# Hfx-J/SGTD

Hardware: AMD Instinct MI355X
Metric: query frames/sec vs map size (descriptor build + candidate selection) (higher is better)
Workload: dtype f64

## Files before the change

### sgtd_amd/csrc/select_kernels.hip.h

```cpp
#pragma once
#include "probe_kernels.hip.h"

#define SGTD_VT_THREADS 1024
#define SGTD_VT_BINS 4096
__host__ __device__ __forceinline__ size_t votes_topk_lds_bytes(u32 frame_span) {
  return (((size_t)frame_span + 3) & ~(size_t)3) * 4 + SGTD_VT_BINS * 4 + SGTD_TOPK_POOL * 8;
}

__global__ __launch_bounds__(SGTD_VT_THREADS) void votes_topk_kernel(QueryView Q, ProbeBuffers B, u32 frame_span, u32 frame_lo,
                                                                      int blocks_per_query, int cand_num, u32 *q_M,
                                                                      unsigned long long *q_P, int *n_cand, int *cand_frame,
                                                                      int *cand_votes, long long *pair_off, u32 *q_pairs) {
  constexpr int NW = SGTD_VT_THREADS / SGTD_WAVE;
  extern __shared__ u32 s_dyn[];
  u32 *s_hist = s_dyn;
  u32 *s_vb = s_dyn + ((frame_span + 3u) & ~3u);
  u64 *s_pool = reinterpret_cast<u64 *>(s_vb + SGTD_VT_BINS);
  __shared__ u32 s_pre[NW][32];
  __shared__ u32 s_ptr[NW][32];
  __shared__ u32 s_cnt[NW][32];
  __shared__ u32 s_M, s_thr, s_n_ge, s_npool;
  __shared__ unsigned long long s_P;
  __shared__ u64 s_red[NW];
  __shared__ int s_picked;
// ... 14 lines not shown
    }
    if (lane == 0) {
      atomicAdd(&s_M, total);
      atomicAdd(&s_P, (unsigned long long)visits);
    }
  }
  __syncthreads();
  u32 *votes = B.votes + (size_t)q * frame_span;
  for (u32 f = tid; f < frame_span; f += SGTD_VT_THREADS) {
    const u32 v = s_hist[f];
    votes[f] = v;
    if (v >= 5) atomicAdd(&s_vb[min(v, (u32)SGTD_VT_BINS - 1u)], 1u);
  }
  if (tid == 0) {
    atomicAdd(&q_M[q], s_M);
    atomicAdd(&q_P[q], s_P);
  }
  __syncthreads();
  if (tid < SGTD_WAVE) {
    constexpr int PER = SGTD_VT_BINS / SGTD_WAVE;
    u32 mine = 0;
    for (int b = 0; b < PER; b++) mine += s_vb[lane * PER + b];
    u32 suffix = mine;
#pragma unroll
    for (int d = 1; d < SGTD_WAVE; d <<= 1) {
      const u32 o = __shfl_down(suffix, d);
      if (lane + d < SGTD_WAVE) suffix += o;
    }
    const u64 okmask = __ballot(suffix >= (u32)cand_num);
    const u32 n_ge = __shfl(suffix, 0);
    if (okmask) {
      const int L = 63 - __builtin_clzll(okmask);
      if (lane == L) {
        u32 acc = suffix - mine;
        int b = L * PER + PER - 1;
        for (; b >= L * PER; b--) { acc += s_vb[b]; if (acc >= (u32)cand_num) break; }
        s_thr = (u32)max(b, 5); s_n_ge = acc;
      }
    } else if (lane == 0) { s_thr = 5; s_n_ge = n_ge; }
  }
  __syncthreads();
  const u32 thr = s_thr;
  int *cf = cand_frame + (size_t)q * cand_num, *cv = cand_votes + (size_t)q * cand_num;
  long long *po = pair_off + (size_t)q * (cand_num + 1);
  if (s_n_ge <= (u32)SGTD_TOPK_POOL) {
    for (u32 f = tid; f < frame_span; f += SGTD_VT_THREADS) {
      const u32 v = s_hist[f];
      if (v >= thr) s_pool[atomicAdd(&s_npool, 1u)] = ((u64)v << 32) | (u64)(0xFFFFFFFFu - f);
    }
    __syncthreads();
    if (tid < SGTD_WAVE) {
      constexpr int PER = SGTD_TOPK_POOL / SGTD_WAVE;
      const u32 np = s_npool;
      u64 a[PER];
#pragma unroll
      for (int k = 0; k < PER; k++) a[k] = ((u32)(k * SGTD_WAVE + lane) < np) ? s_pool[k * SGTD_WAVE + lane] : 0ull;
      int picked = 0;
      u32 acc = 0;
      for (int round = 0; round < cand_num; round++) {
        u64 best = 0;
#pragma unroll
        for (int k = 0; k < PER; k++) best = a[k] > best ? a[k] : best;
#pragma unroll
        for (int dlt = SGTD_WAVE / 2; dlt > 0; dlt >>= 1) {
          const u64 o = __shfl_xor(best, dlt);
          best = o > best ? o : best;
        }
        if ((u32)(best >> 32) < 5u) break;
#pragma unroll
        for (int k = 0; k < PER; k++) a[k] = (a[k] == best) ? 0ull : a[k];
        if (lane == 0) {
          const u32 f = 0xFFFFFFFFu - (u32)(best & 0xFFFFFFFFu);
          cf[picked] = (int)(f + frame_lo);
          cv[picked] = (int)(u32)(best >> 32);
          po[picked] = (long long)acc;
        }
        acc += (u32)(best >> 32);
        picked++;
      }
      if (lane == 0) {
        n_cand[q] = picked;
        q_pairs[q] = acc;
        for (int k = picked; k < cand_num; k++) { cf[k] = -1; cv[k] = 0; }
        for (int k = picked; k <= cand_num; k++) po[k] = (long long)acc;
      }
    }
    return;
  }
  u32 acc = 0;
  for (int round = 0; round < cand_num; round++) {
    u64 best = 0;
    for (u32 f = tid; f < frame_span; f += SGTD_VT_THREADS) {
      const u64 key = ((u64)s_hist[f] << 32) | (u64)(0xFFFFFFFFu - f);
      best = key > best ? key : best;
    }
#pragma unroll
    for (int dlt = SGTD_WAVE / 2; dlt > 0; dlt >>= 1) {
      const u64 o = __shfl_xor(best, dlt);
      best = o > best ? o : best;
    }
    if (lane == 0) s_red[wid] = best;
    __syncthreads();
    if (tid == 0) {
      u64 b = s_red[0];
      for (int w = 1; w < NW; w++) b = s_red[w] > b ? s_red[w] : b;
      const u32 v = (u32)(b >> 32);
      if (v >= 5) {
        const u32 f = 0xFFFFFFFFu - (u32)(b & 0xFFFFFFFFu);
        s_hist[f] = 0;
        cf[s_picked] = (int)(f + frame_lo);
        cv[s_picked] = (int)v;
        po[s_picked] = (long long)acc;
        acc += v;
        s_picked++;
      } else {
        s_picked |= 0x40000000;
      }
    }
    __syncthreads();
    if (s_picked & 0x40000000) break;
  }
  if (tid == 0) {
    const int picked = s_picked & 0x3FFFFFFF;
    n_cand[q] = picked;
    q_pairs[q] = acc;
    for (int k = picked; k < cand_num; k++) { cf[k] = -1; cv[k] = 0; }
    for (int k = picked; k <= cand_num; k++) po[k] = (long long)acc;
  }
}

__global__ __launch_bounds__(256) void cand_prefix_kernel(const int *n_cand, const int *cand_votes, int cand_num, int n_queries,
                                                          long long *pair_off, u32 *q_pairs) {
  const int q = blockIdx.x * blockDim.x + threadIdx.x;
  if (q >= n_queries) return;
  const int nc = n_cand[q];
  u32 acc = 0;
  for (int k = 0; k <= cand_num; k++) {
    pair_off[(size_t)q * (cand_num + 1) + k] = (long long)acc;
    if (k < nc) acc += (u32)cand_votes[(size_t)q * cand_num + k];
  }
  q_pairs[q] = acc;
}

#ifndef SGTD_PQ_THREADS
#define SGTD_PQ_THREADS 512
#endif
#define SGTD_PQ_WAVES (SGTD_PQ_THREADS / SGTD_WAVE)
#ifndef SGTD_PQ_WORDS
#define SGTD_PQ_WORDS 4
#endif
#ifndef SGTD_PQ_OCC
#define SGTD_PQ_OCC 4
#endif
#define SGTD_PQ_TILE_QUADS (SGTD_PQ_WAVES * SGTD_PQ_WORDS * SGTD_WAVE)
#define SGTD_PQ_WAVE_RECS (SGTD_PQ_WORDS * SGTD_WAVE * 4)
#define SGTD_PQ_TILE_RECS (SGTD_PQ_WAVES * SGTD_PQ_WAVE_RECS)
#define SGTD_PQ_DESCS SGTD_PQ_THREADS
#define SGTD_PQ_RANK_BITS (SGTD_PQ_DESCS <= 512 ? 17 : 16)
static_assert(SGTD_PQ_DESCS <= 1024 && SGTD_MAX_CAND <= 64, "an image word holds 6 slot bits and 26 - RANK_BITS descriptor bits");
static_assert(SGTD_PQ_WAVE_RECS * 4 >= 4 * 64 * 8 && (SGTD_PQ_WAVES & (SGTD_PQ_WAVES - 1)) == 0 && SGTD_PQ_WAVES >= 2,
              "a wave's region of the image holds the ranking masks of four dense words; image positions rotate over a power of two of regions");

struct __attribute__((aligned(16))) PqList { u32 pre, first, n, desc; };

template <bool SLOT_TABLE>
__global__ __launch_bounds__(SGTD_PQ_THREADS) __attribute__((amdgpu_waves_per_eu(SGTD_PQ_OCC, SGTD_PQ_OCC))) void pairs_query_kernel(QueryView Q, ProbeBuffers B, const int *n_cand,
                                                                       const int *cand_frame, int cand_num,
                                                                       const long long *pair_off, const u32 *q_pair_base,
                                                                       u64 *pairs, IdMap map, u32 frame_span, u32 frame_lo,
                                                                       const u64 *keep) {
  constexpr int NW = SGTD_PQ_WAVES, QW = SGTD_PQ_WORDS;
  extern __shared__ __attribute__((aligned(16))) u32 s_img[];
  unsigned char *s_slot8 = reinterpret_cast<unsigned char *>(s_img + SGTD_PQ_TILE_RECS);
  __shared__ PqList s_ne[SGTD_PQ_DESCS];
  __shared__ u32 s_start[SGTD_PQ_DESCS + SGTD_WAVE + 8];
  __shared__ u32 s_cnt[NW][64];
  __shared__ u32 s_scan[NW + 1];
  __shared__ u64 s_cand[SGTD_CAND_HASH];
  if (B.overflow()[0] || B.overflow()[1]) return;
  const int tid = threadIdx.x, lane = lane_id(), wid = tid >> 6;
  const int q = blockIdx.x;
  const u32 cnt = Q.count[q];
  const int nc = n_cand[q];
  if (nc == 0 || cnt == 0) return;
  const u64 kept = keep ? keep[q] : ~0ull;
  if (kept == 0) return;
  if (SLOT_TABLE) {
    for (u32 f = tid; f < (((frame_span + 15u) & ~15u) + 16u) / 4u; f += SGTD_PQ_THREADS) reinterpret_cast<u32 *>(s_slot8)[f] = 0xFFFFFFFFu;
    __syncthreads();
    if (tid < nc && ((kept >> tid) & 1ull)) s_slot8[(u32)cand_frame[(size_t)q * cand_num + tid] - frame_lo] = (unsigned char)tid;
  } else {
    s_cand[tid & (SGTD_CAND_HASH - 1)] = SGTD_CAND_EMPTY;
    __syncthreads();
    if (tid < nc && ((kept >> tid) & 1ull)) {
      const u32 f = (u32)cand_frame[(size_t)q * cand_num + tid];
      u32 h = (f * 0x9E3779B1u) >> 24;
      while (atomicCAS(&s_cand[h], SGTD_CAND_EMPTY, ((u64)f << 8) | (u64)tid) != SGTD_CAND_EMPTY) h = (h + 1) & (SGTD_CAND_HASH - 1);
    }
  }
  u32 out_next = 0, first_of_slot = 0;
  if (lane < nc) {
    out_next = q_pair_base[q] + (u32)pair_off[(size_t)q * (cand_num + 1) + lane];
    first_of_slot = map.frame_first[(u32)cand_frame[(size_t)q * cand_num + lane] - map.frame_lo];
  }
  const u32 id_bits = B.id_bits, rank_mask = (1u << id_bits) - 1u;
  const u64 lane_bit = 1ull << lane;
  u32 *my_img = s_img + wid * SGTD_PQ_WAVE_RECS;
  for (u32 sb0 = 0; sb0 < cnt; sb0 += SGTD_PQ_DESCS) {
    __syncthreads();
    u32 n = 0, p = 0;
    if (sb0 + tid < cnt) {
      const uint2 lp = B.list[(long long)q * Q.stride + sb0 + tid];
      p = lp.x; n = lp.y;
    }
    u32 RQ, K;
    const u32 pre = block_excl_scan((n + 3u) >> 2, s_scan, RQ);
    const u32 kx = block_excl_scan(n ? 1u : 0u, s_scan, K);
    if (n) { s_ne[kx] = PqList{pre, p, n, (u32)tid}; s_start[kx] = pre; }
    if ((u32)tid >= K) s_start[tid] = 0xFFFFFFFFu;
    if (tid < SGTD_WAVE + 8) s_start[SGTD_PQ_DESCS + tid] = 0xFFFFFFFFu;
    static_assert(SGTD_PQ_THREADS >= SGTD_WAVE + 8, "the end markers behind the list starts are written by the first 72 threads");
    __syncthreads();
    if (RQ == 0) continue;
    const u32 n_tiles = (RQ + SGTD_PQ_TILE_QUADS - 1) / SGTD_PQ_TILE_QUADS;
    uint4 nrec[QW];
    u32 nk[QW], ndd[QW];
    auto fetch = [&](u32 t) {
      const u32 r0 = t * SGTD_PQ_TILE_QUADS + (u32)wid * (QW * SGTD_WAVE);
      u32 below = 0;
#pragma unroll
      for (int i = 0; i < SGTD_PQ_DESCS / SGTD_WAVE; i++) below += s_start[i * SGTD_WAVE + lane] <= r0 ? 1u : 0u;
      const u32 k0 = wave_sum(below) - 1u;
      const u32 st = s_start[k0 + 1u + (u32)lane];
      u32 kl[QW];
      u32 c_prev = 0;
      bool slow = false;
#pragma unroll
      for (int u = 0; u < QW; u++) {
        const u32 w_lo = r0 + (u32)u * SGTD_WAVE;
        const u32 c = (u32)__builtin_popcountll(__builtin_amdgcn_ballot_w64(st <= w_lo + SGTD_WAVE));
        u64 marks = 0;
        for (u32 i = c_prev; i < c; i++) marks |= 1ull << ((u32)__builtin_amdgcn_readlane((int)st, (int)i) - 1u - w_lo);
        kl[u] = k0 + c_prev + __builtin_amdgcn_mbcnt_hi((u32)(marks >> 32), __builtin_amdgcn_mbcnt_lo((u32)marks, 0u));
        c_prev = c;
        slow = slow || c >= (u32)SGTD_WAVE;
      }
      if (slow) {
#pragma unroll
        for (int u = 0; u < QW; u++) {
          const u32 r = r0 + (u32)u * SGTD_WAVE + (u32)lane;
          u32 lo = 0, hi = K;
          while (hi - lo > 1u) {
            const u32 mid = (lo + hi) >> 1;
            if (s_start[mid] <= r) lo = mid; else hi = mid;
          }
          kl[u] = lo;
        }
      }
#pragma unroll
      for (int u = 0; u < QW; u++) {
        const u32 r = r0 + (u32)u * SGTD_WAVE + (u32)lane;
        const PqList L = s_ne[min(kl[u], K - 1u)];
        const bool ok = r < RQ;
        const u32 quad = r - L.pre;
        nk[u] = ok ? min(4u, L.n - (quad << 2)) : 0u;
        ndd[u] = L.desc << SGTD_PQ_RANK_BITS;
        nrec[u] = *reinterpret_cast<const uint4 *>(B.rec_at(ok ? L.first + quad : 0u));
      }
    };
    fetch(0);
    for (u32 t = 0; t < n_tiles; t++) {
      uint4 rc[QW];
      u32 kk[QW], dd[QW];
#pragma unroll
      for (int u = 0; u < QW; u++) { rc[u] = nrec[u]; kk[u] = nk[u]; dd[u] = ndd[u]; }
      if (t + 1 < n_tiles) fetch(t + 1);
#if defined(SGTD_EXP_PQ) && SGTD_EXP_PQ == 2
      {
        u32 x = 0;
        for (int u = 0; u < QW; u++) x ^= rc[u].x ^ rc[u].y ^ rc[u].z ^ rc[u].w ^ kk[u] ^ dd[u];
        if (x == 0x12345678u) pairs[0] = x;
        continue;
      }
#endif
      u32 nd = 0;
      static_assert(QW % 2 == 0, "the candidates of two quad-words are counted by one wave scan (16-bit halves)");
#pragma unroll
      for (int u0 = 0; u0 < QW; u0 += 2) {
        u32 sl[2][4], mine[2] = {0, 0};
#pragma unroll
        for (int h = 0; h < 2; h++) {
          const int u = u0 + h;
          const u32 w4[4] = {rc[u].x, rc[u].y, rc[u].z, rc[u].w};
#pragma unroll
          for (int i = 0; i < 4; i++) {
            const u32 lf = w4[i] >> id_bits;
            if (SLOT_TABLE) {
              sl[h][i] = (u32)s_slot8[min(lf, frame_span)];
              sl[h][i] = (u32)i < kk[u] ? sl[h][i] : 0xFFu;
            } else {
              sl[h][i] = 0xFFu;
              if ((u32)i < kk[u] && lf < frame_span) sl[h][i] = cand_slot(s_cand, lf + frame_lo);
            }
            mine[h] += sl[h][i] != 0xFFu ? 1u : 0u;
          }
        }
        const u32 both = mine[0] | (mine[1] << 16);
        const u32 inc = wave_incl_scan(both);
        const u32 tot2 = (u32)__builtin_amdgcn_readlane((int)inc, SGTD_WAVE - 1);
        u32 at[2] = {nd + ((inc - both) & 0xFFFFu), nd + (tot2 & 0xFFFFu) + ((inc - both) >> 16)};
#pragma unroll
        for (int h = 0; h < 2; h++) {
          const int u = u0 + h;
          const u32 w4[4] = {rc[u].x, rc[u].y, rc[u].z, rc[u].w};
#pragma unroll
          for (int i = 0; i < 4; i++)
            if (sl[h][i] != 0xFFu) my_img[at[h]++] = (sl[h][i] << 26) | dd[u] | (w4[i] & rank_mask);
        }
        nd += (tot2 & 0xFFFFu) + (tot2 >> 16);
      }
#if defined(SGTD_EXP_PQ) && SGTD_EXP_PQ == 3
      if (nd == 0xFFFFFFFFu) pairs[0] = 0;
      continue;
#endif
      __builtin_amdgcn_wave_barrier();
      constexpr int MAXD = SGTD_PQ_WAVE_RECS / SGTD_WAVE, GRP = 4;
      u32 dw[MAXD], rk[MAXD];
      const u32 ndw = (nd + SGTD_WAVE - 1) / SGTD_WAVE;
#pragma unroll
      for (int g0 = 0; g0 < MAXD; g0 += GRP) {
#pragma unroll
        for (int w = g0; w < g0 + GRP; w++) { dw[w] = 0xFFFFFFFFu; rk[w] = 0; }
        if ((u32)g0 < ndw) {
#pragma unroll
          for (int w = g0; w < g0 + GRP; w++) {
            const u32 v = my_img[w * SGTD_WAVE + lane];
            dw[w] = (u32)(w * SGTD_WAVE + lane) < nd ? v : 0xFFFFFFFFu;
          }
        }
      }
      u32 run_s = 0;
      u64 *m = reinterpret_cast<u64 *>(my_img);
#pragma unroll
      for (int g0 = 0; g0 < MAXD; g0 += GRP) {
        if ((u32)g0 < ndw) {
          __builtin_amdgcn_wave_barrier();
#pragma unroll
          for (int w = 0; w < GRP; w++) m[w * SGTD_WAVE + lane] = 0;
          __builtin_amdgcn_wave_barrier();
#pragma unroll
          for (int w = 0; w < GRP; w++)
            if (dw[g0 + w] != 0xFFFFFFFFu) atomicOr(&m[w * SGTD_WAVE + (dw[g0 + w] >> 26)], lane_bit);
          __builtin_amdgcn_wave_barrier();
#pragma unroll
          for (int w = 0; w < GRP; w++) {
            const u64 own = m[w * SGTD_WAVE + lane];
            const u32 s = (dw[g0 + w] >> 26) & 63u;
            const u64 gm = m[w * SGTD_WAVE + s];
            const u32 before = (u32)__builtin_amdgcn_ds_bpermute((int)(s << 2), (int)run_s);
            rk[g0 + w] = before + __builtin_amdgcn_mbcnt_hi((u32)(gm >> 32), __builtin_amdgcn_mbcnt_lo((u32)gm, 0u));
            run_s += (u32)__builtin_popcountll(own);
          }
        }
      }
      s_cnt[wid][lane] = run_s;
      __syncthreads();
#if defined(SGTD_EXP_PQ) && SGTD_EXP_PQ == 4
      if (rk[0] == 0xFFFFFFF1u) pairs[0] = 0;
      continue;
#endif
      u32 tot = 0, mine_before = 0;
#pragma unroll
      for (int w = 0; w < NW; w++) {
        const u32 c = s_cnt[w][lane];
        mine_before += w < wid ? c : 0u;
        tot += c;
      }
      const u32 slot_inc = wave_incl_scan(tot);
      const u32 slot_off = slot_inc - tot;
      const u32 n_img = (u32)__builtin_amdgcn_readlane((int)slot_inc, SGTD_WAVE - 1);
      const u32 my_base = slot_off + mine_before;
#pragma unroll
      for (int g0 = 0; g0 < MAXD; g0 += GRP) {
        if ((u32)g0 < ndw) {
#pragma unroll
          for (int w = g0; w < g0 + GRP; w++) {
            const u32 pos = (u32)__builtin_amdgcn_ds_bpermute((int)((dw[w] >> 26) << 2), (int)my_base) + rk[w];
            if (dw[w] != 0xFFFFFFFFu)
              s_img[((pos >> 6) & (NW - 1)) * SGTD_PQ_WAVE_RECS + (((pos >> 6) / NW) << 6) + (pos & 63u)] = dw[w];
          }
        }
      }
      __syncthreads();
#if defined(SGTD_EXP_PQ) && SGTD_EXP_PQ == 5
      out_next += tot;
      continue;
#endif
      for (u32 c = (u32)wid; c * SGTD_WAVE < n_img; c += NW) {
        const u32 e = c * SGTD_WAVE + lane;
        const bool ok = e < n_img;
        const u32 wv = my_img[((c / NW) << 6) + lane];
        const u32 s4 = ok ? (wv >> 26) << 2 : 0u;
        const u32 o = (u32)__builtin_amdgcn_ds_bpermute((int)s4, (int)(out_next - slot_off));
        u32 g = (u32)__builtin_amdgcn_ds_bpermute((int)s4, (int)first_of_slot) + (wv & ((1u << SGTD_PQ_RANK_BITS) - 1u));
        if (ok) {
          if (map.by_frame) g = map.by_frame[g];
#if defined(SGTD_EXP_PQ) && SGTD_EXP_PQ == 1
          if (g == 0xFFFFFFF3u)
#endif
          pairs[o + e] = ((u64)(sb0 + ((wv >> SGTD_PQ_RANK_BITS) & (SGTD_PQ_DESCS - 1u))) << 32) | (u64)g;
        }
      }
      out_next += tot;
      __builtin_amdgcn_wave_barrier();
    }
  }
}
```

### sgtd_amd/csrc/sgtd_accel.hip

```cpp
#include "../../include/sgtd_accel.h"

#include <hip/hip_runtime.h>

#include <algorithm>
#include <atomic>
#include <chrono>
#include <cmath>
#include <cstdio>
#include <cstring>
#include <limits>
#include <memory>
#include <string>
#include <vector>

#include "build_kernel.hip.h"
#include "common.hip.h"
#include "table_kernels.hip.h"
#include "probe_kernels.hip.h"
#include "select_kernels.hip.h"
#include "verify_kernels.hip.h"
#include "verify_mfma.hip.h"
#include "exchange_kernels.hip.h"
#include "remove_kernels.hip.h"
#include "filter_kernels.hip.h"
// ... 727 lines not shown
  }
  frame_first_kernel<<<grid_for(E, 256), 256, 0, e->stream>>>(key, E, lo, e->frame_first.as<u32>());
  HIPCHK(hipGetLastError());
  frame_longest_kernel<<<grid_for(E, 256), 256, 0, e->stream>>>(key, E, lo, e->frame_first.as<u32>(), e->longest.as<u32>());
  HIPCHK(hipGetLastError());
  HIPCHK(hipMemcpyAsync(h, e->longest.p, sizeof(u32), hipMemcpyDeviceToHost, e->stream));
  HIPCHK(hipStreamSynchronize(e->stream));
  u32 need = 1;
  while (need < 32 && (1ull << need) < (unsigned long long)h[0]) need++;
  auto fits = [&](u32 b) { return b < 32 && (unsigned long long)span < (1ull << (32 - b)) - 1ull; };
  if (bits < need || !fits(bits)) {
    bits = std::max<u32>(need, 13);
    if (!fits(bits)) bits = need;
    if (!fits(bits)) {
      e->err = "a 32-bit entry id cannot hold this table's frame span and its largest frame";
      return SGTD_ERR_UNSUPPORTED;
    }
  }
  if (e->id_by_frame) {
    id_of_sorted_kernel<<<grid_for(E, 256), 256, 0, e->stream>>>(key, e->by_frame.as<u32>(), E, lo, e->frame_first.as<u32>(), bits,
                                                                 e->id_of_g.as<u32>());
    HIPCHK(hipGetLastError());
  }
  return SGTD_OK;
}

int do_finalize(sgtd_engine *e, bool force_merge = false) {
  if (e->finalized && !(force_merge && e->n_seg > 1)) return SGTD_OK;
  if (e->attached_to) { e->err = "the table belongs to another handle (sgtd_attach_table): only its owner rebuilds it"; return SGTD_ERR_STATE; }
  e->table_version++;
  const long long E = e->n_entries;
  if (E >= (1ll << 32) - 2 - SGTD_SENTINELS) return SGTD_ERR_UNSUPPORTED;
  const auto t0 = std::chrono::steady_clock::now();
  sgtd_engine::Segment &M = e->seg[0], &T = e->seg[1];
  const long long tail_max = e->tail_max > 0 ? (long long)e->tail_max : std::max<long long>(262144, (M.g1 - M.g0) / 8);
  u32 bits = 0;
  CHK(build_idmap(e, bits));
  const bool can_tail = !force_merge && M.built && M.g0 == 0 && M.g1 > 0 && M.g1 <= E && E - M.g1 <= tail_max &&
                        bits == e->id_bits && !e->id_by_frame && (E == M.g1 || e->append_min_frame > M.frame_hi);
  e->id_bits = bits;
  if (can_tail) {
    if (E > M.g1) { CHK(build_segment(e, T, M.g1, E)); e->n_seg = 2; }
    else { T.built = false; e->n_seg = 1; }
  } else {
    CHK(build_segment(e, M, 0, E));
    T.built = false; T.g0 = T.g1 = E;
    e->n_seg = 1;
    e->append_min_frame = 0xFFFFFFFFu;
  }
  e->ms_finalize = std::chrono::duration<float, std::milli>(std::chrono::steady_clock::now() - t0).count();
  e->finalized = true;
  return SGTD_OK;
}

int rec_alloc(sgtd_engine *e, bool compact_lists) {
#ifdef SGTD_EXP_SHADOW16
  CHK(ensure(e, e->rec, (e->rec_cap + 16) * sizeof(u32) * 3 / 2 + 256));
#else
  CHK(ensure(e, e->rec, (e->rec_cap + 16) * sizeof(u32)));
#endif
  if (compact_lists) CHK(ensure(e, e->c_pair, std::min(e->rec_cap, kIndexLimit) * sizeof(u64)));
  if (e->diag) {
    CHK(ensure(e, e->rec_cell, e->rec_cap));
    CHK(ensure(e, e->rec_dis, e->rec_cap * sizeof(double)));
  }
  CHK(ensure(e, e->pairs, e->pair_cap * sizeof(u64)));
  CHK(ensure(e, e->amb_queue, std::max<size_t>(65536, e->rec_cap / 64) * sizeof(uint2)));
  return SGTD_OK;
}

u32 block_chunk(const sgtd_engine *e) {
  if (const char *o = getenv("SGTD_BLOCK_CHUNK")) { const int c = atoi(o); if (c == 32 || c == 64 || c == 128) return (u32)c; }
  u32 c = SGTD_PROBE_CHUNK;
  while (c > SGTD_SUB_DESCS && (long long)e->nq * ((e->q_stride + c - 1) / c) < 1024) c >>= 1;
  return c;
}

struct Views {
  TableView T;
  QueryView Q;
  ProbeBuffers B;
  u32 span;
  int blocks_per_query;
};

Views make_views(sgtd_engine *e) {
  Views v;
  v.span = e->have_frames ? (e->frame_hi - e->frame_lo + 1) : 1;
  TableView &T = v.T;
  const sgtd_engine::Segment &S = e->seg[0], &S1 = e->seg[1];
  T.ent = S.hot.as<HotEntry>(); T.map = id_map(e, e->id_bits ? e->id_bits : 13); T.cold_side = e->tab.side.as<double>();
  T.dir = S.dir.as<BucketDir>();
  T.hash = S.hash.as<HashSlot>(); T.hash_mask = S.hash_mask;
  T.coarse_at = e->coarse_at; T.whole_at = e->whole_at;
  T.n_entries = (u32)(S.g1 - S.g0); T.frame_lo = e->have_frames ? e->frame_lo : 0; T.frame_span = v.span;
  T.tail_off = e->n_seg > 1 ? T.n_entries + SGTD_SENTINELS : 0u;
  T.dir1 = S1.dir.as<BucketDir>(); T.hash1 = S1.hash.as<HashSlot>(); T.hash_mask1 = S1.hash_mask;
  T.n_entries1 = e->n_seg > 1 ? (u32)(S1.g1 - S1.g0) : 0u;
  QueryView &Q = v.Q;
  Q.side = e->qd.side.as<double>(); Q.qrec = e->qd.qrec.as<QueryRec>();
  Q.label = e->qd.label.as<int>(); Q.frame = e->qd.frame.as<u32>();
  Q.count = e->q_count.as<u32>(); Q.stride = e->q_stride; Q.n_queries = e->nq; Q.chunk = block_chunk(e);
  ProbeBuffers &B = v.B;
  B.rec_cell = e->rec_cell.as<unsigned char>(); B.rec_dis = e->rec_dis.as<double>();
  B.rec_cap = (u32)std::min<size_t>(e->rec_cap >> SGTD_REC_SHIFT, kIndexLimit);
  B.rec = e->rec.as<u32>(); B.id_bits = e->id_bits ? e->id_bits : 13;
  B.ctr = e->cursors.as<u32>();
  {
    const size_t streams = (size_t)e->n_cus * 32 * SGTD_PAIR;
    u32 slab = SGTD_REC_SLAB;
    while (slab > 512u && (size_t)slab * streams * 4 > e->rec_cap) slab >>= 1;
    if (const char *o = getenv("SGTD_REC_SLAB")) slab = (u32)std::max(512, atoi(o));
    B.rec_slab = slab >> SGTD_REC_SHIFT;
  }
  {
    const double per_pass = SGTD_PAIR >= 4 ? 3.2 : (SGTD_PAIR >= 2 ? 1.9 : 1.0);
    B.rec_rate = 64;
    if (e->stats.last_P_swept > 0 && e->stats.last_M > 0) {
      const double meas = 256.0 * (double)e->stats.last_M / ((double)e->stats.last_P_swept * per_pass);
      const double scale = e->stats.last_queries > 0 ? (double)e->nq / (double)e->stats.last_queries : 1.0;
      const double fit = 256.0 * (0.6 * (double)e->rec_cap - 256.0 * (double)e->stats.last_D * scale) /
                         std::max(1.0, (double)e->stats.last_P_swept * scale * per_pass);
      const double want = std::max(std::min(3.0 * meas, fit), 1.2 * meas);
      B.rec_rate = (u32)std::min(256.0, std::max(want < 16.0 && fit < 16.0 ? 2.0 : 16.0, std::ceil(want)));
    }
    B.rec_rate = std::min(B.rec_rate, e->rec_rate_cap);
    if (e->diag) B.rec_rate = 256;
    if (e->rec_rate_hook) B.rec_rate = e->rec_rate_hook;
  }
  B.amb_queue = e->amb_queue.as<uint2>();
  B.amb_cap = (u32)std::min<size_t>(e->amb_queue.bytes / sizeof(uint2), 0xFFFFFFF0u);
  B.list = e->list.as<uint2>(); B.n_visit = e->n_visit.as<u32>();
  B.votes = e->votes.as<u32>();
  v.blocks_per_query = (int)((e->q_stride + block_chunk(e) - 1) / block_chunk(e));
  return v;
}

int launch_block_write(sgtd_engine *e, const Views &v, const CompactLists &CL, int agrid, int blocks) {
  const int cn = e->dc.cand_num;
  if (v.T.map.bits <= SGTD_NARROW_RANK_BITS && !e->wide_pairs)
    block_write_kernel<true><<<agrid, 256, 0, e->stream>>>(v.Q, v.B, CL, blocks, e->blk_count.as<u32>(), cn, e->pair_off.as<long long>(),
                                                            e->q_pair_base.as<u32>(), e->pairs.as<u64>(), v.T.map, e->n_cand.as<int>(),
                                                            e->cand_frame.as<int>());
  else
    block_write_kernel<false><<<agrid, 256, 0, e->stream>>>(v.Q, v.B, CL, blocks, e->blk_count.as<u32>(), cn, e->pair_off.as<long long>(),
                                                             e->q_pair_base.as<u32>(), e->pairs.as<u64>(), v.T.map, e->n_cand.as<int>(),
                                                             e->cand_frame.as<int>());
  HIPCHK(hipGetLastError());
  return SGTD_OK;
}

int launch_pairs_query(sgtd_engine *e, const Views &v, const u64 *keep = nullptr) {
  const int cn = e->dc.cand_num;
  const size_t img = (size_t)SGTD_PQ_TILE_RECS * sizeof(u32);
  const size_t tab = (((size_t)v.span + 15) & ~(size_t)15) + 16;
  static const size_t room = lds_room(&pairs_query_kernel<true>);
  if (img + tab <= room) {
    HIPCHK(hipFuncSetAttribute(reinterpret_cast<const void *>(&pairs_query_kernel<true>), hipFuncAttributeMaxDynamicSharedMemorySize, (int)(img + tab)));
    pairs_query_kernel<true><<<e->nq, SGTD_PQ_THREADS, img + tab, e->stream>>>(v.Q, v.B, e->n_cand.as<int>(), e->cand_frame.as<int>(), cn,
                                                                                e->pair_off.as<long long>(), e->q_pair_base.as<u32>(),
                                                                                e->pairs.as<u64>(), v.T.map, v.span, v.T.frame_lo, keep);
  } else {
    pairs_query_kernel<false><<<e->nq, SGTD_PQ_THREADS, img, e->stream>>>(v.Q, v.B, e->n_cand.as<int>(), e->cand_frame.as<int>(), cn,
                                                                           e->pair_off.as<long long>(), e->q_pair_base.as<u32>(),
                                                                           e->pairs.as<u64>(), v.T.map, v.span, v.T.frame_lo, keep);
  }
  HIPCHK(hipGetLastError());
  return SGTD_OK;
}

int export_candidates(sgtd_engine *e, const Views &v) {
  if (!e->export_packed) return SGTD_OK;
  const int nq = e->nq, cn = e->dc.cand_num;
  if (xchg_packed_ints(nq, cn) > e->export_cap) {
    e->err = "the registered candidate-export buffer is too small for this batch";
    return SGTD_ERR_CAPACITY;
  }
  if (e->export_busy) {
    HIPCHK(hipStreamWaitEvent(e->stream, e->ev_export_free, 0));
    e->export_busy = false;
  }
  export_candidates_kernel<<<std::min(grid_for((long long)nq * cn, 256), 512), 256, 0, e->stream>>>(
      e->cand_frame.as<int>(), e->cand_votes.as<int>(), v.B.overflow(), nq, cn, ++e->batch_serial, e->export_packed);
  HIPCHK(hipGetLastError());
  HIPCHK(hipEventRecord(e->ev_cand, e->stream));
  return SGTD_OK;
}

int launch_lists(sgtd_engine *e, const Views &v, const u64 *keep, bool first) {
  const int nq = e->nq, cn = e->dc.cand_num;
  if (keep) {
    cand_prefix_masked_kernel<<<grid_for(nq, 256), 256, 0, e->stream>>>(e->n_cand.as<int>(), e->cand_votes.as<int>(), keep, cn, nq,
                                                                          e->pair_off.as<long long>(), e->q_pairs.as<u32>());
    HIPCHK(hipGetLastError());
  } else if (!e->fused_votes_last || e->lists_masked) {
    cand_prefix_kernel<<<grid_for(nq, 256), 256, 0, e->stream>>>(e->n_cand.as<int>(), e->cand_votes.as<int>(), cn, nq,
                                                                   e->pair_off.as<long long>(), e->q_pairs.as<u32>());
    HIPCHK(hipGetLastError());
  }
  e->lists_masked = keep != nullptr;
  e->list_keep = keep;
  if (e->timing && first) HIPCHK(hipEventRecord(e->ev[EV_COUNT_T], e->stream));
  if (!first) HIPCHK(hipMemsetAsync(v.B.overflow() + 1, 0, sizeof(int), e->stream));
  query_base_kernel<<<1, 256, 0, e->stream>>>(e->q_pairs.as<u32>(), e->q_pair_base.as<u32>(), nq,
                                               (u32)std::min<size_t>(e->pair_cap, 0xFFFFFFF0u), v.B.overflow());
  HIPCHK(hipGetLastError());
  if (e->timing && first) HIPCHK(hipEventRecord(e->ev[EV_SCAN], e->stream));
  CHK(launch_pairs_query(e, v, keep));
  if (e->timing && first) HIPCHK(hipEventRecord(e->ev[EV_WRITE], e->stream));
  if (first) {
    batch_totals_kernel<<<1, 1, 0, e->stream>>>(v.B.ctr, e->totals.as<unsigned long long>());
    HIPCHK(hipGetLastError());
  }
  e->lists_pending = false;
  e->verified = false;
  e->batch_synced = false;
  return SGTD_OK;
}

int rebase_filter(sgtd_engine *e, u32 frame_lo, u32 span, int n_rows, DevBuf &dst) {
  const FrameFilter &F = *e->batch_filt;
  const size_t words = ((size_t)span + 63) / 64;
  e->filt_host.assign((size_t)n_rows * words, 0ull);
  const long long shift = (long long)frame_lo - (long long)F.lo;
  const u64 last = span % 64 ? (1ull << (span % 64)) - 1ull : ~0ull;
  for (int r = 0; r < n_rows; r++) {
    u64 *dst = e->filt_host.data() + (size_t)r * words;
    for (size_t w = 0; w < words; w++) dst[w] = row_bits_at(F.row(r), F.words, shift + (long long)w * 64);
    dst[words - 1] &= last;
  }
  CHK(ensure(e, dst, e->filt_host.size() * sizeof(u64)));
  CHK(h2d(e, dst.p, e->filt_host.data(), e->filt_host.size() * sizeof(u64)));
  return SGTD_OK;
}

int prepare_filter(sgtd_engine *e, u32 frame_lo, u32 span) {
  const FrameFilter &F = *e->batch_filt;
  if (e->filt_rows.p && F.serial == e->filt_rows_serial && frame_lo == e->filt_rows_lo && span == e->filt_rows_span) return SGTD_OK;
  CHK(rebase_filter(e, frame_lo, span, F.n_rows == 1 ? 1 : e->nq, e->filt_rows));
  e->filt_rows_serial = F.serial; e->filt_rows_lo = frame_lo; e->filt_rows_span = span;
  e->prior_rows_valid = false;
  return SGTD_OK;
}

static int batch_row_count(const sgtd_engine *e) {
  const bool per_q = (e->batch_filt && e->batch_filt->n_rows > 1) || (e->batch_prior && e->batch_prior->n_rows > 1);
  return per_q ? e->nq : 1;
}

int prepare_prior(sgtd_engine *e, u32 frame_lo, u32 span) {
  const PositionPrior &P = *e->batch_prior;
  const int n_rows = batch_row_count(e);
  const sgtd_engine::PriorKey key{P.serial, e->poses_serial, e->batch_filt ? e->batch_filt->serial : 0ull, frame_lo, span, n_rows};
  if (e->filt_rows.p && e->prior_rows_valid && key == e->prior_key) return SGTD_OK;
  if (!e->pos_dev.p || e->pos_serial != e->poses_serial || e->pos_lo != frame_lo || e->pos_span != span) {
    e->pos_host.assign(span, make_float4(0.f, 0.f, 0.f, 0.f));
    const size_t n_ids = e->has_pose.size();
    for (u32 f = 0; f < span; f++) {
      const size_t id = (size_t)frame_lo + f;
      if (id >= n_ids) break;
      if (e->has_pose[id]) {
        const float *m = e->poses.data() + id * 12;
        e->pos_host[f] = make_float4(m[3], m[7], m[11], 1.f);
      }
    }
    CHK(ensure(e, e->pos_dev, (size_t)span * sizeof(float4)));
    CHK(h2d(e, e->pos_dev.p, e->pos_host.data(), (size_t)span * sizeof(float4)));
    e->pos_serial = e->poses_serial; e->pos_lo = frame_lo; e->pos_span = span;
  }
  CHK(ensure(e, e->prior_dev, P.prm.size() * sizeof(double4)));
  CHK(h2d(e, e->prior_dev.p, P.prm.data(), P.prm.size() * sizeof(double4)));
  const u64 *base = nullptr;
  int base_rows = 1;
  if (e->batch_filt) {
    const FrameFilter &F = *e->batch_filt;
    base_rows = F.n_rows == 1 ? 1 : e->nq;
    if (!e->filt_base.p || F.serial != e->filt_base_serial || frame_lo != e->filt_base_lo || span != e->filt_base_span) {
      CHK(rebase_filter(e, frame_lo, span, base_rows, e->filt_base));
      e->filt_base_serial = F.serial; e->filt_base_lo = frame_lo; e->filt_base_span = span;
    }
    base = e->filt_base.as<u64>();
  }
  const u32 words = (span + 63) / 64;
  CHK(ensure(e, e->filt_rows, (size_t)n_rows * words * sizeof(u64)));
  const long long waves = (long long)n_rows * words;
  const int grid = (int)((waves + SGTD_PRIOR_THREADS / SGTD_WAVE - 1) / (SGTD_PRIOR_THREADS / SGTD_WAVE));
  prior_rows_kernel<<<grid, SGTD_PRIOR_THREADS, 0, e->stream>>>(e->pos_dev.as<float4>(), span, words, e->prior_dev.as<double4>(),
                                                               P.n_rows == 1 ? 1 : n_rows, P.dims, base, base_rows, n_rows, e->filt_rows.as<u64>());
  HIPCHK(hipGetLastError());
  e->prior_key = key; e->prior_rows_valid = true;
  e->filt_rows_serial = 0;
  return SGTD_OK;
}

int launch_filter(sgtd_engine *e, const Views &v) {
  const int nq = e->nq, n_rows = batch_row_count(e);
  const u32 words = (v.span + 63) / 64;
  const long long chunks = (e->q_stride + SGTD_WAVE - 1) / SGTD_WAVE;
  const int want = (int)std::max<long long>(1, ((long long)e->n_cus * 8 + nq - 1) / nq);
  const int wg_per_q = (int)std::max<long long>(1, std::min<long long>(want, (chunks + SGTD_FILT_WAVES - 1) / SGTD_FILT_WAVES));
  const int grid = nq * wg_per_q;
  const size_t lds = (size_t)words * sizeof(u64);
  const u64 *rows = e->filt_rows.as<u64>();
  if (e->diag) {
    if (lds <= 65536) filter_compact_kernel<true><<<grid, SGTD_FILT_THREADS, lds, e->stream>>>(v.Q, v.B, rows, n_rows, words, v.span, wg_per_q);
    else filter_compact_kernel<false><<<grid, SGTD_FILT_THREADS, 0, e->stream>>>(v.Q, v.B, rows, n_rows, words, v.span, wg_per_q);
  } else {
    if (lds <= 65536)
      filter_records_kernel<true><<<grid, SGTD_FILT_THREADS, lds, e->stream>>>(v.Q, v.B, rows, n_rows, words, v.span, wg_per_q, e->q_M.as<u32>());
    else
      filter_records_kernel<false><<<grid, SGTD_FILT_THREADS, 0, e->stream>>>(v.Q, v.B, rows, n_rows, words, v.span, wg_per_q, e->q_M.as<u32>());
  }
  HIPCHK(hipGetLastError());
  return SGTD_OK;
}

int launch_select(sgtd_engine *e) {
  const int nq = e->nq;
// ... 2114 lines not shown
```

Baseline: 187,700.

## Batch several load rounds per pairs-query sort with larger per-wave LDS regions

The pairs-query kernel can now gather matching records from several load rounds into an enlarged per-wave LDS region before running one ranking and scatter pass, instead of sorting after every tile. It picks the number of rounds per query from the expected match density, and falls back to a single-round re-sort if any wave's region overflows. This targets the fixed sort, barrier and scatter cost paid per tile. In exchange it adds a per-query pre-pass summing list lengths, more LDS per block (possibly lower occupancy), and overflow-retry complexity.

```diff
diff --git a/sgtd_amd/csrc/select_kernels.hip.h b/sgtd_amd/csrc/select_kernels.hip.h
--- a/sgtd_amd/csrc/select_kernels.hip.h
+++ b/sgtd_amd/csrc/select_kernels.hip.h
@@ -190,14 +190,27 @@
 #ifndef SGTD_PQ_OCC
 #define SGTD_PQ_OCC 4
 #endif
-#define SGTD_PQ_TILE_QUADS (SGTD_PQ_WAVES * SGTD_PQ_WORDS * SGTD_WAVE)
+#ifndef SGTD_PQ_ROUNDS
+#define SGTD_PQ_ROUNDS 4
+#endif
+#define SGTD_PQ_ROUND_QUADS (SGTD_PQ_WAVES * SGTD_PQ_WORDS * SGTD_WAVE)
 #define SGTD_PQ_WAVE_RECS (SGTD_PQ_WORDS * SGTD_WAVE * 4)
+#ifndef SGTD_PQ_REGION
+#define SGTD_PQ_REGION (SGTD_PQ_ROUNDS > 1 ? 1280 : SGTD_PQ_WAVE_RECS)
+#endif
 #define SGTD_PQ_TILE_RECS (SGTD_PQ_WAVES * SGTD_PQ_WAVE_RECS)
 #define SGTD_PQ_DESCS SGTD_PQ_THREADS
 #define SGTD_PQ_RANK_BITS (SGTD_PQ_DESCS <= 512 ? 17 : 16)
 static_assert(SGTD_PQ_DESCS <= 1024 && SGTD_MAX_CAND <= 64, "an image word holds 6 slot bits and 26 - RANK_BITS descriptor bits");
 static_assert(SGTD_PQ_WAVE_RECS * 4 >= 4 * 64 * 8 && (SGTD_PQ_WAVES & (SGTD_PQ_WAVES - 1)) == 0 && SGTD_PQ_WAVES >= 2,
               "a wave's region of the image holds the ranking masks of four dense words; image positions rotate over a power of two of regions");
+static_assert(SGTD_PQ_REGION >= SGTD_PQ_WAVE_RECS && SGTD_PQ_REGION % (4 * SGTD_WAVE) == 0 && SGTD_PQ_ROUNDS >= 1,
+              "a region holds one load round whatever its records are (the one-round tiles of a re-sort cannot overflow); the ranking works on groups of four dense words");
+
+__host__ __device__ __forceinline__ u32 pq_rounds(u32 region, u64 pairs, u64 recs) {
+  const u64 r = (2ull * region * recs) / (3ull * SGTD_PQ_WAVE_RECS * (pairs ? pairs : 1ull));
+  return (u32)(r < 1 ? 1 : r > (u64)SGTD_PQ_ROUNDS ? (u64)SGTD_PQ_ROUNDS : r);
+}
 
 struct __attribute__((aligned(16))) PqList { u32 pre, first, n, desc; };
 
@@ -206,10 +219,11 @@
                                                                        const int *cand_frame, int cand_num,
                                                                        const long long *pair_off, const u32 *q_pair_base,
                                                                        u64 *pairs, IdMap map, u32 frame_span, u32 frame_lo,
-                                                                       const u64 *keep) {
+                                                                       const u64 *keep, u32 region) {
   constexpr int NW = SGTD_PQ_WAVES, QW = SGTD_PQ_WORDS;
+  constexpr u32 WQ = QW * SGTD_WAVE;
   extern __shared__ __attribute__((aligned(16))) u32 s_img[];
-  unsigned char *s_slot8 = reinterpret_cast<unsigned char *>(s_img + SGTD_PQ_TILE_RECS);
+  unsigned char *s_slot8 = reinterpret_cast<unsigned char *>(s_img + NW * region);
   __shared__ PqList s_ne[SGTD_PQ_DESCS];
   __shared__ u32 s_start[SGTD_PQ_DESCS + SGTD_WAVE + 8];
   __shared__ u32 s_cnt[NW][64];
@@ -236,6 +250,13 @@
       while (atomicCAS(&s_cand[h], SGTD_CAND_EMPTY, ((u64)f << 8) | (u64)tid) != SGTD_CAND_EMPTY) h = (h + 1) & (SGTD_CAND_HASH - 1);
     }
   }
+  u32 rounds_q = 1;
+  if (SGTD_PQ_ROUNDS > 1) {
+    u32 mine = 0, recs;
+    for (u32 d = tid; d < cnt; d += SGTD_PQ_THREADS) mine += B.list[(long long)q * Q.stride + d].y;
+    (void)block_excl_scan(mine, s_scan, recs);
+    rounds_q = pq_rounds(region, (u64)pair_off[(size_t)q * (cand_num + 1) + cand_num], (u64)recs);
+  }
   u32 out_next = 0, first_of_slot = 0;
   if (lane < nc) {
     out_next = q_pair_base[q] + (u32)pair_off[(size_t)q * (cand_num + 1) + lane];
@@ -243,7 +264,7 @@
   }
   const u32 id_bits = B.id_bits, rank_mask = (1u << id_bits) - 1u;
   const u64 lane_bit = 1ull << lane;
-  u32 *my_img = s_img + wid * SGTD_PQ_WAVE_RECS;
+  u32 *my_img = s_img + wid * region;
   for (u32 sb0 = 0; sb0 < cnt; sb0 += SGTD_PQ_DESCS) {
     __syncthreads();
     u32 n = 0, p = 0;
@@ -260,11 +281,15 @@
     static_assert(SGTD_PQ_THREADS >= SGTD_WAVE + 8, "the end markers behind the list starts are written by the first 72 threads");
     __syncthreads();
     if (RQ == 0) continue;
-    const u32 n_tiles = (RQ + SGTD_PQ_TILE_QUADS - 1) / SGTD_PQ_TILE_QUADS;
     uint4 nrec[QW];
     u32 nk[QW], ndd[QW];
-    auto fetch = [&](u32 t) {
-      const u32 r0 = t * SGTD_PQ_TILE_QUADS + (u32)wid * (QW * SGTD_WAVE);
+    auto fetch = [&](u32 r0) {
+      r0 = (u32)__builtin_amdgcn_readfirstlane((int)r0);
+      if (r0 >= RQ) {
+#pragma unroll
+        for (int u = 0; u < QW; u++) { nk[u] = 0; ndd[u] = 0; nrec[u] = make_uint4(0, 0, 0, 0); }
+        return;
+      }
       u32 below = 0;
 #pragma unroll
       for (int i = 0; i < SGTD_PQ_DESCS / SGTD_WAVE; i++) below += s_start[i * SGTD_WAVE + lane] <= r0 ? 1u : 0u;
@@ -306,63 +331,86 @@
         nrec[u] = *reinterpret_cast<const uint4 *>(B.rec_at(ok ? L.first + quad : 0u));
       }
     };
-    fetch(0);
-    for (u32 t = 0; t < n_tiles; t++) {
-      uint4 rc[QW];
-      u32 kk[QW], dd[QW];
-#pragma unroll
-      for (int u = 0; u < QW; u++) { rc[u] = nrec[u]; kk[u] = nk[u]; dd[u] = ndd[u]; }
-      if (t + 1 < n_tiles) fetch(t + 1);
+    auto rounds_at = [&](u32 t0, u32 resort) {
+      return resort ? 1u : min(rounds_q, (RQ - t0 + SGTD_PQ_ROUND_QUADS - 1u) / SGTD_PQ_ROUND_QUADS);
+    };
+    u32 T0 = 0, resort = 0;
+    u32 R = rounds_at(0, 0);
+    fetch((u32)wid * R * WQ);
+    while (T0 < RQ) {
+      const u32 T1 = T0 + R * SGTD_PQ_ROUND_QUADS;
+      const u32 resort1 = resort ? resort - 1u : 0u;
+      const u32 R1 = T1 < RQ ? rounds_at(T1, resort1) : 1u;
+      u32 nd = 0;
+      bool full = false;
 #if defined(SGTD_EXP_PQ) && SGTD_EXP_PQ == 2
+      u32 x = 0;
+#endif
+      for (u32 r = 0; r < R; r++) {
+        uint4 rc[QW];
+        u32 kk[QW], dd[QW];
+#pragma unroll
+        for (int u = 0; u < QW; u++) { rc[u] = nrec[u]; kk[u] = nk[u]; dd[u] = ndd[u]; }
+        if (r + 1 < R) fetch(T0 + ((u32)wid * R + r + 1u) * WQ);
+        else if (T1 < RQ) fetch(T1 + (u32)wid * R1 * WQ);
+#if defined(SGTD_EXP_PQ) && SGTD_EXP_PQ == 2
+        for (int u = 0; u < QW; u++) x ^= rc[u].x ^ rc[u].y ^ rc[u].z ^ rc[u].w ^ kk[u] ^ dd[u];
+        continue;
+#endif
+        static_assert(QW % 2 == 0, "the candidates of two quad-words are counted by one wave scan (16-bit halves)");
+#pragma unroll
+        for (int u0 = 0; u0 < QW; u0 += 2) {
+          u32 sl[2][4], mine[2] = {0, 0};
+#pragma unroll
+          for (int h = 0; h < 2; h++) {
+            const int u = u0 + h;
+            const u32 w4[4] = {rc[u].x, rc[u].y, rc[u].z, rc[u].w};
+#pragma unroll
+            for (int i = 0; i < 4; i++) {
+              const u32 lf = w4[i] >> id_bits;
+              if (SLOT_TABLE) {
+                sl[h][i] = (u32)s_slot8[min(lf, frame_span)];
+                sl[h][i] = (u32)i < kk[u] ? sl[h][i] : 0xFFu;
+              } else {
+                sl[h][i] = 0xFFu;
+                if ((u32)i < kk[u] && lf < frame_span) sl[h][i] = cand_slot(s_cand, lf + frame_lo);
+              }
+              mine[h] += sl[h][i] != 0xFFu ? 1u : 0u;
+            }
+          }
+          const u32 both = mine[0] | (mine[1] << 16);
+          const u32 inc = wave_incl_scan(both);
+          const u32 tot2 = (u32)__builtin_amdgcn_readlane((int)inc, SGTD_WAVE - 1);
+          const u32 add = (tot2 & 0xFFFFu) + (tot2 >> 16);
+          full = full || nd + add > region;
+          if (!full) {
+            u32 at[2] = {nd + ((inc - both) & 0xFFFFu), nd + (tot2 & 0xFFFFu) + ((inc - both) >> 16)};
+#pragma unroll
+            for (int h = 0; h < 2; h++) {
+              const int u = u0 + h;
+              const u32 w4[4] = {rc[u].x, rc[u].y, rc[u].z, rc[u].w};
+#pragma unroll
+              for (int i = 0; i < 4; i++)
+                if (sl[h][i] != 0xFFu) my_img[at[h]++] = (sl[h][i] << 26) | dd[u] | (w4[i] & rank_mask);
+            }
+            nd += add;
+          }
+        }
+      }
+#if defined(SGTD_EXP_PQ) && (SGTD_EXP_PQ == 2 || SGTD_EXP_PQ == 3)
       {
-        u32 x = 0;
-        for (int u = 0; u < QW; u++) x ^= rc[u].x ^ rc[u].y ^ rc[u].z ^ rc[u].w ^ kk[u] ^ dd[u];
+#if SGTD_EXP_PQ == 2
         if (x == 0x12345678u) pairs[0] = x;
+#else
+        if (nd == 0xFFFFFFFFu) pairs[0] = 0;
+#endif
+        T0 = T1; R = R1; resort = resort1;
         continue;
       }
 #endif
-      u32 nd = 0;
-      static_assert(QW % 2 == 0, "the candidates of two quad-words are counted by one wave scan (16-bit halves)");
-#pragma unroll
-      for (int u0 = 0; u0 < QW; u0 += 2) {
-        u32 sl[2][4], mine[2] = {0, 0};
-#pragma unroll
-        for (int h = 0; h < 2; h++) {
-          const int u = u0 + h;
-          const u32 w4[4] = {rc[u].x, rc[u].y, rc[u].z, rc[u].w};
-#pragma unroll
-          for (int i = 0; i < 4; i++) {
-            const u32 lf = w4[i] >> id_bits;
-            if (SLOT_TABLE) {
-              sl[h][i] = (u32)s_slot8[min(lf, frame_span)];
-              sl[h][i] = (u32)i < kk[u] ? sl[h][i] : 0xFFu;
-            } else {
-              sl[h][i] = 0xFFu;
-              if ((u32)i < kk[u] && lf < frame_span) sl[h][i] = cand_slot(s_cand, lf + frame_lo);
-            }
-            mine[h] += sl[h][i] != 0xFFu ? 1u : 0u;
-          }
-        }
-        const u32 both = mine[0] | (mine[1] << 16);
-        const u32 inc = wave_incl_scan(both);
-        const u32 tot2 = (u32)__builtin_amdgcn_readlane((int)inc, SGTD_WAVE - 1);
-        u32 at[2] = {nd + ((inc - both) & 0xFFFFu), nd + (tot2 & 0xFFFFu) + ((inc - both) >> 16)};
-#pragma unroll
-        for (int h = 0; h < 2; h++) {
-          const int u = u0 + h;
-          const u32 w4[4] = {rc[u].x, rc[u].y, rc[u].z, rc[u].w};
-#pragma unroll
-          for (int i = 0; i < 4; i++)
-            if (sl[h][i] != 0xFFu) my_img[at[h]++] = (sl[h][i] << 26) | dd[u] | (w4[i] & rank_mask);
-        }
-        nd += (tot2 & 0xFFFFu) + (tot2 >> 16);
-      }
-#if defined(SGTD_EXP_PQ) && SGTD_EXP_PQ == 3
-      if (nd == 0xFFFFFFFFu) pairs[0] = 0;
-      continue;
-#endif
+      if (full) nd = 0;
       __builtin_amdgcn_wave_barrier();
-      constexpr int MAXD = SGTD_PQ_WAVE_RECS / SGTD_WAVE, GRP = 4;
+      constexpr int MAXD = SGTD_PQ_REGION / SGTD_WAVE, GRP = 4;
       u32 dw[MAXD], rk[MAXD];
       const u32 ndw = (nd + SGTD_WAVE - 1) / SGTD_WAVE;
 #pragma unroll
@@ -401,18 +449,26 @@
           }
         }
       }
-      s_cnt[wid][lane] = run_s;
+      s_cnt[wid][lane] = full ? 0x80000000u : run_s;
       __syncthreads();
 #if defined(SGTD_EXP_PQ) && SGTD_EXP_PQ == 4
       if (rk[0] == 0xFFFFFFF1u) pairs[0] = 0;
+      T0 = T1; R = R1; resort = resort1;
       continue;
 #endif
-      u32 tot = 0, mine_before = 0;
+      u32 tot = 0, mine_before = 0, any = 0;
 #pragma unroll
       for (int w = 0; w < NW; w++) {
         const u32 c = s_cnt[w][lane];
+        any |= c;
         mine_before += w < wid ? c : 0u;
         tot += c;
+      }
+      if (__builtin_amdgcn_readfirstlane(any) >> 31) {
+        __syncthreads();
+        resort = R; R = 1;
+        fetch(T0 + (u32)wid * WQ);
+        continue;
       }
       const u32 slot_inc = wave_incl_scan(tot);
       const u32 slot_off = slot_inc - tot;
@@ -425,13 +481,14 @@
           for (int w = g0; w < g0 + GRP; w++) {
             const u32 pos = (u32)__builtin_amdgcn_ds_bpermute((int)((dw[w] >> 26) << 2), (int)my_base) + rk[w];
             if (dw[w] != 0xFFFFFFFFu)
-              s_img[((pos >> 6) & (NW - 1)) * SGTD_PQ_WAVE_RECS + (((pos >> 6) / NW) << 6) + (pos & 63u)] = dw[w];
+              s_img[((pos >> 6) & (NW - 1)) * region + (((pos >> 6) / NW) << 6) + (pos & 63u)] = dw[w];
           }
         }
       }
       __syncthreads();
 #if defined(SGTD_EXP_PQ) && SGTD_EXP_PQ == 5
       out_next += tot;
+      T0 = T1; R = R1; resort = resort1;
       continue;
 #endif
       for (u32 c = (u32)wid; c * SGTD_WAVE < n_img; c += NW) {
@@ -451,6 +508,7 @@
       }
       out_next += tot;
       __builtin_amdgcn_wave_barrier();
+      T0 = T1; R = R1; resort = resort1;
     }
   }
 }
diff --git a/sgtd_amd/csrc/sgtd_accel.hip b/sgtd_amd/csrc/sgtd_accel.hip
--- a/sgtd_amd/csrc/sgtd_accel.hip
+++ b/sgtd_amd/csrc/sgtd_accel.hip
@@ -903,18 +903,26 @@
 
 int launch_pairs_query(sgtd_engine *e, const Views &v, const u64 *keep = nullptr) {
   const int cn = e->dc.cand_num;
-  const size_t img = (size_t)SGTD_PQ_TILE_RECS * sizeof(u32);
   const size_t tab = (((size_t)v.span + 15) & ~(size_t)15) + 16;
-  static const size_t room = lds_room(&pairs_query_kernel<true>);
-  if (img + tab <= room) {
+  static const size_t room = lds_room(&pairs_query_kernel<true>), room_hash = lds_room(&pairs_query_kernel<false>);
+  auto region_for = [](size_t dyn_rest, size_t kernel_room) {
+    const size_t big = (size_t)SGTD_PQ_WAVES * SGTD_PQ_REGION * sizeof(u32);
+    return (u32)(kernel_room < 150 * 1024 && 2 * (160 * 1024 - kernel_room + big + dyn_rest) <= 160 * 1024 ? SGTD_PQ_REGION : SGTD_PQ_WAVE_RECS);
+  };
+  if ((size_t)SGTD_PQ_TILE_RECS * sizeof(u32) + tab <= room) {
+    const u32 region = region_for(tab, room);
+    const size_t img = (size_t)SGTD_PQ_WAVES * region * sizeof(u32);
     HIPCHK(hipFuncSetAttribute(reinterpret_cast<const void *>(&pairs_query_kernel<true>), hipFuncAttributeMaxDynamicSharedMemorySize, (int)(img + tab)));
     pairs_query_kernel<true><<<e->nq, SGTD_PQ_THREADS, img + tab, e->stream>>>(v.Q, v.B, e->n_cand.as<int>(), e->cand_frame.as<int>(), cn,
                                                                                 e->pair_off.as<long long>(), e->q_pair_base.as<u32>(),
-                                                                                e->pairs.as<u64>(), v.T.map, v.span, v.T.frame_lo, keep);
+                                                                                e->pairs.as<u64>(), v.T.map, v.span, v.T.frame_lo, keep, region);
   } else {
+    const u32 region = region_for(0, room_hash);
+    const size_t img = (size_t)SGTD_PQ_WAVES * region * sizeof(u32);
+    HIPCHK(hipFuncSetAttribute(reinterpret_cast<const void *>(&pairs_query_kernel<false>), hipFuncAttributeMaxDynamicSharedMemorySize, (int)img));
     pairs_query_kernel<false><<<e->nq, SGTD_PQ_THREADS, img, e->stream>>>(v.Q, v.B, e->n_cand.as<int>(), e->cand_frame.as<int>(), cn,
                                                                            e->pair_off.as<long long>(), e->q_pair_base.as<u32>(),
-                                                                           e->pairs.as<u64>(), v.T.map, v.span, v.T.frame_lo, keep);
+                                                                           e->pairs.as<u64>(), v.T.map, v.span, v.T.frame_lo, keep, region);
   }
   HIPCHK(hipGetLastError());
   return SGTD_OK;
```

Result: no change. 186,200 (-0.8%).
